# pingooio/pingoo

Hardware: AMD Instinct MI355X
Metric: requests/sec matched (whole node), 1k-rule WAF (higher is better)
Workload: dtype u8

## Files before the change

include/pwaf.h:

```cpp
#ifndef PWAF_H
#define PWAF_H

#include <stddef.h>
#include <stdint.h>

#ifdef __cplusplus
extern "C" {
#endif

#define PWAF_ABI_VERSION 4u

#define PWAF_OK 0
#define PWAF_E_INVALID_ARG (-1)
#define PWAF_E_SYNTAX (-2)
#define PWAF_E_UNSUPPORTED (-3)
#define PWAF_E_LIST (-4)
#define PWAF_E_DEVICE (-5)
#define PWAF_E_BATCH (-6)
#define PWAF_E_NOMEM (-7)
#define PWAF_E_BUSY (-8)
#define PWAF_W_PARTIAL 1

#define PWAF_ACTION_ALLOW 0u
#define PWAF_ACTION_BLOCK 1u
// ... 49 lines not shown
void pwaf_list_free(char **items, size_t n);

#define PWAF_OPT_NO_UA_GATE 1u
#define PWAF_OPT_NO_CAPTCHA_BYPASS 2u
#define PWAF_OPT_STRICT 8u
#define PWAF_OPT_LENIENT 32u
#define PWAF_OPT_GLOBAL_VERDICT_TABLES 128u
#define PWAF_OPT_SPARSE_VERDICT 16384u
#define PWAF_OPT_DENSE_VERDICT 2048u
#define PWAF_OPT_TINY_VERDICT_SLOTS 4096u
#define PWAF_OPT_NO_DENSE_SWITCH 65536u
#define PWAF_OPT_EAGER_CMP 32768u
#define PWAF_OPT_NO_DIR_SUMMARY 8192u
#define PWAF_OPT_GEO_ANSWERS 256u
#define PWAF_OPT_RULE_HITS 131072u
#define PWAF_OPT_NO_RESIDUAL 64u
#define PWAF_OPT_NO_RESIDUAL_JIT 1024u
#define PWAF_OPT_NO_PREFILTER 4u
#define PWAF_OPT_FILTER_STRIDE2 16u
#define PWAF_OPT_NO_CONFIRM 512u
typedef struct pwaf_options {
    uint32_t struct_size;
    uint32_t flags;
    int32_t device;
    uint32_t lds_table_budget;
    uint32_t max_dfa_states;
    uint32_t max_table_bytes;
    uint32_t reserved[2];
} pwaf_options;

// ... 238 lines not shown
int pwaf_engine_stats(const pwaf_engine *, pwaf_stats *out);
int pwaf_engine_rule_errors(pwaf_engine *, uint64_t *counts, size_t n_rules);
int pwaf_engine_residual_mode(const pwaf_engine *);
const char *pwaf_engine_residual_fallback(const pwaf_engine *);
size_t pwaf_program_residual_source(const pwaf_program *, int kind, char *buf, size_t cap);
long pwaf_program_residual_compile(const pwaf_program *, const char *arch, char *err, size_t err_len);
int pwaf_program_confirm_field(const pwaf_program *, uint32_t group, const uint8_t *bytes, size_t len, uint32_t arena_offset,
                               uint16_t *atoms, size_t cap, size_t *n_atoms, int *flagged, int *walk);
int pwaf_program_confirm_shape(const pwaf_program *, uint32_t group, uint32_t out[8]);
size_t pwaf_program_flat_image(const pwaf_program *, uint32_t group, uint32_t tier, uint8_t *buf, size_t cap);
#define PWAF_LIST_SCAN_WORDS 16
int pwaf_program_list_scans(const pwaf_program *, uint32_t *out, size_t cap, size_t *n_descs);
uint32_t pwaf_engine_compute_units(const pwaf_engine *);
int pwaf_engine_address_tables(const pwaf_engine *, uint32_t out[8]);
int pwaf_engine_coarse_tables(const pwaf_engine *, uint32_t out[16]);
int pwaf_program_stats(const pwaf_program *, pwaf_stats *out);

size_t pwaf_derive_path(const uint8_t *uri_path, size_t len);
void pwaf_derive_user_agent(const uint8_t *hdr, size_t len, int present, size_t *out_start, size_t *out_len);
void pwaf_derive_host(const uint8_t *uri_host, size_t uri_host_len, int uri_host_present,
                      const uint8_t *host_hdr, size_t host_hdr_len, int host_hdr_present,
                      int *out_from_header, size_t *out_start, size_t *out_len);

const char *pwaf_last_error(void);
uint32_t pwaf_abi_version(void);

#ifdef __cplusplus
}
#endif
#endif
// ... 1 lines not shown
```

pingoo_amd/_abi.py:

```python
import ctypes as C

ABI_VERSION = 4

OK = 0
E_INVALID_ARG = -1
E_SYNTAX = -2
E_UNSUPPORTED = -3
E_LIST = -4
E_DEVICE = -5
E_BATCH = -6
E_NOMEM = -7
E_BUSY = -8

ACTION_ALLOW, ACTION_BLOCK, ACTION_CAPTCHA, ACTION_BYPASS = 0, 1, 2, 3
RULE_NONE = 0xFFFFFFFF
RULE_UA_GATE = 0xFFFFFFFE
RULE_CAPTCHA_ENDPOINT = 0xFFFFFFFD
RULE_ACTION_BLOCK, RULE_ACTION_CAPTCHA = 1, 2

LIST_STRING, LIST_INT, LIST_IP = 0, 1, 2
OPT_NO_UA_GATE, OPT_NO_CAPTCHA_BYPASS, OPT_NO_PREFILTER, OPT_STRICT, OPT_FILTER_STRIDE2, OPT_LENIENT, OPT_NO_RESIDUAL, OPT_GLOBAL_VERDICT_TABLES, OPT_NO_CONFIRM, OPT_NO_RESIDUAL_JIT = 1, 2, 4, 8, 16, 32, 64, 128, 512, 1024
OPT_DENSE_VERDICT, OPT_TINY_VERDICT_SLOTS, OPT_NO_DIR_SUMMARY, OPT_SPARSE_VERDICT, OPT_EAGER_CMP, OPT_NO_DENSE_SWITCH = 2048, 4096, 8192, 16384, 32768, 65536
OPT_GEO_ANSWERS = 256
OPT_RULE_HITS = 131072
W_PARTIAL = 1
MEM_HOST, MEM_DEVICE = 0, 1
FLAG_CAPTCHA_VERIFIED = 1
ROUTE_NONE = 0xFFFFFFFF
RECORD_NONE = 0xFFFFFFFF
N_FIELDS = 5
FIELD_NAMES = ("host", "url", "path", "method", "user_agent")
ARENA_PAD = 16
ADDRESS_TABLE_FIELDS = ("escapes", "n_vals", "has_summary", "shift", "common", "packed", "classes", "sets")
CONFIRM_SHAPE_FIELDS = ("entries", "bytes", "class_words", "in_lds", "longest", "top_class_pos", "widest_bin", "has_walk")
LIST_SCAN_FIELDS = ("phase", "pass", "tier", "threads", "hot_bytes", "n_hot", "n_delta", "behind_filter", "merge_rec", "dense_mode", "share_owner", "need_bit",
                    "launch", "launch_count", "wg_per_cu", "zero15")
FLAT_SHAPE_FIELDS = ("n_states", "n_classes", "scalar_mode", "ill_class", "n_full", "n_delta", "lds_bytes")
COARSE_TABLE_FIELDS = ("present", "shift", "bytes", "blocks_set", "summary_blocks_set", "threads", "wg_per_cu", "zero7",
                       "rec_present", "rec_shift", "rec_bytes", "rec_blocks_set", "zero12", "zero13", "zero14", "zero15")
GEO_ANSWER_TABLE_FIELDS = ("has_table", "escapes", "n_vals", "has_summary", "shift", "common", "records", "zero")


class RuleDesc(C.Structure):
    _fields_ = [
        ("name", C.c_char_p),
        ("expression", C.c_char_p),
        ("actions", C.POINTER(C.c_uint8)),
        ("n_actions", C.c_uint32),
        ("reserved", C.c_uint32),
    ]


class RouteDesc(C.Structure):

# ... 201 lines not shown
```

pingoo_amd/csrc/engine.cpp:

```cpp
#include <hip/hip_runtime_api.h>

#include <cstdio>
#include <algorithm>
#include <cstring>
#include <map>
#include <memory>
#include <mutex>
#include <string>
#include <type_traits>
#include <unordered_map>
#include <vector>

#include "dirtable.h"
#include "georec.h"
#include "frontend.h"
#include "kernels.h"
#include "lscan_split.h"
#include "program.h"
#include "records.h"
#include "scanplan.h"
#include "tableplan.h"

using namespace pwaf;

// ... 157 lines not shown

struct Scratch {
    std::mutex mu;
    hipStream_t stream = nullptr, side = nullptr;
    hipEvent_t ev_fork = nullptr, ev_join = nullptr, done = nullptr;
    bool used = false;
    hipStream_t last = nullptr;
    bool last_own = false;
    DevBuf status;
    uint64_t pool_entries = 0;
    struct View { void *p = nullptr; };
    View res_cols;
    bool retry = false;
    DevBuf err_sink;
    DevBuf ipres;
    DevBuf rec, pool, gate_lists, attr;
    DevBuf verdict_spill;
    DevBuf res_words;
    DevBuf zero_block;
    View ctrl, cand_bits, visit_bits, walk_bits;
    DevBuf chunk_bits, cand_cnt;
    DevBuf need;
    DevBuf pairs;
    DevBuf zero_off;
    static constexpr uint32_t kArgSlots = 8;
    DevBuf args;
    PinBuf arg_slot[kArgSlots];
    hipEvent_t arg_ev[kArgSlots] = {};
    bool arg_pending[kArgSlots] = {};
    uint32_t arg_next = 0;
// ... 29 lines not shown
            if (ev) (void)hipEventDestroy(ev);
    }
};
static constexpr size_t kContexts = 3;

struct pwaf_engine : PlanShape, PassShape {
    pwaf_program prog;
    int device = 0;
    std::vector<std::unique_ptr<Scratch>> ctx;
    size_t next_ctx = 0;
    std::vector<DevGroup> groups;
    DevBuf num_atoms, bit_atoms , trig_off, trig_rules, always_rules, country_luts , rules, lits, set_masks;
    DevBuf lazy_atoms;
    DevBuf short_atoms;
    DevBuf class_rows, dir_esc, leaf_root, geo_leaf_root;
    DevBuf iu_vals[2], iu_masks[2];
    DevBuf ip_root4, ip_root6, ip_nodes, geo_root4, geo_root6, geo_nodes, geo_recs;
    std::mutex mu;
    std::mutex prof_mu;
    DevBuf residual_errors;
    std::string residual_note;
    JitKernel residual_jit;
    DevBuf rules_unrouted;
    DevBuf residual_blob, geo_rec_root4, geo_rec_root6, geo_rec_nodes;
    DevBuf pass_base, colmask, dir24 , dir_chunks, dir_vals, dir_summary;
    uint32_t dir_sum_shift = 0, dir_common = 0;
    DevBuf dir_coarse;
    uint32_t dir_coarse_shift = 0, dir_coarse_bytes = 0, dir_coarse_set = 0, dir_summary_set = 0;
    uint32_t dir_n_esc = 0, dir_n_vals = 0;
    bool geo_answers = false;
// ... 392 lines not shown
        v.always_rules = (const uint32_t *)e->always_rules.p;
        for (int var = 0; var < 2; var++) {
            v.iu_vals[var] = (const int64_t *)e->iu_vals[var].p;
            v.iu_masks[var] = (const uint32_t *)e->iu_masks[var].p;
            v.iu_n[var] = e->iu_n[var];
            v.iu_words[var] = e->iu_words[var];
        }
        v.country_masks = (const uint32_t *)e->country_luts.p;
        v.cc_words = e->cc_words;
        v.rules = (const DevRule *)e->rules.p;
        v.n_rules = (uint32_t)P.rules.size();
        v.lits = (const uint32_t *)e->lits.p;
        set_trie_args(e, v);
        if ((rc = S.ipres.reserve((size_t)n * (v.ipres_packed ? 4 : 8) + 64))) return rc;
        v.ipres = (uint32_t *)S.ipres.p;
        v.out = d_out;
        v.counts = (unsigned long long *)d_counts;
        v.match_idx = d_match_idx;
        v.n_matches = d_n_matches;
        return PWAF_OK;
    }

    int zero_head_records() {
        for (size_t k = 0; k < e->groups.size(); k++) {
            const DevGroup &d = e->groups[k];
            if (!d.filtered || d.filter.heads.empty()) continue;
            if (slab_count(col_bytes[d.field], slab0_of(d.field)) != 0 && !(sw.filter_debug_skip & 4u)) continue;
            HIP_TRY(hipMemsetAsync((uint32_t *)S.rec.p + k * (size_t)n, 0, (size_t)n * 4, stream));
        }
        return PWAF_OK;
// ... 28 lines not shown
        if (rc || !d_geo) return rc;
        GeoRecArgs ga{};
        set_georec_args(e, ga);
        ga.ip = db.ip;
        ga.ip_is_v6 = db.ip_is_v6;
        ga.asn = db.asn;
        ga.country = db.country;
        ga.n = n;
        ga.out = (uint2 *)d_geo;
        return side_stage(q, "georec", 25ull * n, "georec kernel", [&] { return launch_georec(ga, q); });
    }
    int attr_stage(hipStream_t q) {
        if (attr_launched) return PWAF_OK;
        attr_launched = true;
        if (q == stream && sw.placement == 0) HIP_TRY(hipStreamWaitEvent(stream, S.ev_join, 0));
        return side_stage(q, "attr", 0xFEu, "attribute kernel", [&] { return sw.skip_attr ? (int)hipMemsetAsync(v.ghdr, 0, (size_t)n_groups * 4, q) : launch_attr(v, q); });
    }
    int attr_at_start() {
        int rc;
        if (sw.placement == 0) return ipres_stage(S.side);
        if (sw.placement == 3) return (rc = ipres_stage(S.side)) ? rc : attr_stage(S.side);
        return PWAF_OK;
    }
    int attr_after_filter() {
        int rc;
        switch (sw.placement) {
        case 0: return attr_stage(stream);
        case 1: return (rc = ipres_stage(stream)) ? rc : attr_stage(stream);
        case 2: return (rc = ipres_stage(S.side)) ? rc : attr_stage(S.side);
        default: return PWAF_OK;
        }
// ... 662 lines not shown
    up(e->bit_atoms, t.bit_col);
    up(e->num_atoms, t.cmp_atoms);
    up(e->lazy_atoms, t.lazy_atoms);
    up(e->lits, t.lits);
    up(e->trig_off, t.trig_off);
    up(e->trig_rules, t.trig_rules);
    up(e->always_rules, t.always);
    up(e->country_luts, t.cc_masks);
    up(e->rules, P.rules);
    if (!t.rules_unrouted.empty()) up(e->rules_unrouted, t.rules_unrouted);
    up(e->set_masks, P.set_masks);
    up(e->ip_root4, P.ipset_trie.root4);
    up(e->ip_root6, P.ipset_trie.root6);
    up(e->ip_nodes, P.ipset_trie.nodes);
    up(e->class_rows, t.class_rows);
    up(e->geo_root4, t.geo_root4);
    up(e->geo_root6, t.geo_root6);
    up(e->geo_nodes, t.geo_nodes);
    up(e->leaf_root, std::vector<uint32_t>(65536, TRIE_LEAF));
    up(e->geo_leaf_root, std::vector<uint32_t>(65536, TRIE_LEAF | t.geo_default));
    if (P.n_residual) {
        up(e->residual_blob, P.residual_blob);
        up(e->residual_errors, std::vector<unsigned long long>(P.n_residual, 0ull));
        if (P.has_geo && P.residual_needs_geo) {
            const std::vector<uint32_t> leaf0(65536, TRIE_LEAF);
            up(e->geo_rec_root4, P.geo_trie.root4.empty() ? leaf0 : P.geo_trie.root4);
            up(e->geo_rec_root6, P.geo_trie.root6.empty() ? leaf0 : P.geo_trie.root6);
            up(e->geo_rec_nodes, P.geo_trie.nodes);
            up(e->geo_recs, P.geo_recs);
        }
// ... 241 lines not shown
    out[6] = e->n_classes;
    out[7] = P.set_words ? (uint32_t)(P.set_masks.size() / P.set_words) : 1u;
    return PWAF_OK;
}
int pwaf_engine_coarse_tables(const pwaf_engine *e, uint32_t out[16]) {
    if (!e || !out) return fail(PWAF_E_INVALID_ARG, "pwaf_engine_coarse_tables: NULL argument");
    const IpresShape sh = ipres_shape();
    for (int i = 0; i < 16; i++) out[i] = 0;
    out[0] = e->dir_coarse.p ? 1u : 0u;
    out[1] = e->dir_coarse_shift;
    out[2] = e->dir_coarse_bytes;
    out[3] = e->dir_coarse_set;
    out[4] = e->dir_summary_set;
    out[5] = e->dir_coarse.p ? sh.threads : 256u;
    out[6] = e->dir_coarse.p ? sh.wg_per_cu : 8u;
    return PWAF_OK;
}
int pwaf_engine_geo_answer_tables(const pwaf_engine *e, uint32_t out[8]) {
    if (!e || !out) return fail(PWAF_E_INVALID_ARG, "pwaf_engine_geo_answer_tables: NULL argument");
    if (int rc = need_geo_answers(e, "pwaf_engine_geo_answer_tables")) return rc;
    out[0] = e->georec_chunks.p ? 1u : 0u;
    out[1] = e->georec_n_esc;
    out[2] = e->georec_chunks.p ? e->georec_n_vals : 0u;
    out[3] = e->georec_summary.p ? 1u : 0u;
    out[4] = e->georec_shift;
    out[5] = e->georec_common;
    out[6] = (uint32_t)std::max<size_t>(1, e->prog.p->geo_recs.size());
    out[7] = 0;
    return PWAF_OK;
}
// ... 864 lines not shown
```

pingoo_amd/csrc/kernels.h:

```cpp
#pragma once
#include <cstdint>
#include <string>
#include <vector>

#include "program.h"
#include "scanplan.h"

namespace pwaf {

static constexpr int kMaxPasses = 250;
static constexpr int kVerdictPre = 12;
static constexpr uint32_t kDirChunkWords = 32;

static constexpr uint32_t REC_OVERFLOW = 0x80000000u;
struct PoolEntry {
    uint32_t atom;
    uint32_t next;
};

struct ScanArgs {
    const uint8_t *data;
    const uint32_t *off;
    uint32_t n;
    const uint16_t *tab;
// ... 282 lines not shown
    const uint32_t *dir_summary;
    uint32_t dir_sum_shift, dir_common;
    const uint32_t *dir_coarse;
    uint32_t dir_coarse_shift, dir_coarse_bytes;
    const uint2 *dir_esc;
    const uint32_t *class_rows;
    uint32_t class_words;
    uint32_t acmp_words;
    uint32_t geo_default;
    uint32_t *ipres;
    uint32_t ipres_packed;
    uint32_t has_geo;
    uint4 *gpairs;
    uint32_t *ghdr;
    uint32_t pair_stride;
    uint32_t attr_blocks;
    pwaf_verdict *out;
    unsigned long long *counts;
    uint32_t *match_idx;
    uint32_t *n_matches;
    pwaf_rule_hit *hits;
    uint32_t hits_cap;
    uint32_t *n_hits;
    unsigned long long *rule_hits;
    uint32_t *route;
    uint32_t route_base;
};

int launch_scan(const ScanArgs &a, void *stream);
struct GatedTable {
// ... 36 lines not shown
```

pingoo_amd/csrc/kernels.hip:

```cpp
#include <hip/hip_runtime.h>

#include <cstdlib>
#include <mutex>
#include <set>

#include "confirm.h"
#include "utf8.h"
#include "kernels.h"
#include "residual.h"

namespace pwaf {

static constexpr int kScanThreads = 1024;
static constexpr int kScanWaves = kScanThreads / 64;
static constexpr uint32_t kNone = 0xFFFFFFFFu;

#define PWAF_LDS __attribute__((address_space(3)))
#define PWAF_GLOBAL __attribute__((address_space(1)))
typedef const PWAF_LDS uint16_t *lds_u16_ptr;
typedef const PWAF_GLOBAL uint16_t *glb_u16_ptr;
typedef const PWAF_LDS uint32_t *lds_u32_ptr;
typedef const PWAF_LDS uint8_t *lds_u8_ptr;
typedef unsigned int u32x4 __attribute__((ext_vector_type(4)));
typedef u32x4 u32x4_u __attribute__((aligned(1)));
// ... 2271 lines not shown

    constexpr int kPre = BR == 1 ? 4 : kVerdictPre;
    constexpr int kBitRegs = BR;
    struct Bits {
        unsigned long long w[kBitRegs];
    };
    struct Inputs {
        uint32_t rv[kPre];
        uint32_t base[kPre];
        Bits bits;
        unsigned long long rest[kBitRegs];
        uint32_t flags, n_pairs;
        uint4 pair0;
        uint32_t res0;
        uint32_t lraw[2];
    };
    const uint32_t *my_bits[kBitRegs];
    uint32_t my_base[kBitRegs];
    bool my_live[kBitRegs];
#pragma unroll
    for (int r = 0; r < kBitRegs; r++) {
        const uint32_t ps = (uint32_t)r * 64 + lane;
        my_live[r] = ps < a.n_passes;
        my_bits[r] = nullptr;
        my_base[r] = 0;
        if (my_live[r]) {
            const PassInfo pi = a.passes[ps];
            const uint32_t kind = pi.kind_slot >> 24, sl = pi.kind_slot & 0xFFFFFFu;
            if (kind == 3) my_live[r] = false;
            my_bits[r] = kind == 1 ? a.cand_bits + (size_t)sl * a.bit_words : kind == 2 ? a.visit_bits + (size_t)sl * a.bit_words : nullptr;
// ... 23 lines not shown
                if (ps == kNone && nzp[r] != 0) {
                    const int l = __builtin_ctzll(nzp[r]);
                    nzp[r] &= nzp[r] - 1;
                    ps = (uint32_t)r * 64 + (uint32_t)l;
                    word = ((unsigned long long)(uint32_t)__builtin_amdgcn_readlane((int)(bt.w[r] >> 32), l) << 32) | (uint32_t)__builtin_amdgcn_readlane((int)(uint32_t)bt.w[r], l);
                    base = (uint32_t)__builtin_amdgcn_readlane((int)my_base[r], l);
                }
            }
            in.base[q] = base;
            in.rv[q] = (ps != kNone && valid && ((word >> lane) & 1ull)) ? a.rec[(size_t)ps * a.n + i] : 0u;
        }
#pragma unroll
        for (int r = 0; r < kBitRegs; r++) in.rest[r] = nzp[r];
        in.bits = bt;
        in.flags = valid ? (uint32_t)a.flags[i] : 0u;
        const uint32_t gg = min(g, a.n_groups - 1);
        {
            const uint32_t *src = a.ghdr + gg;
#pragma unroll
            for (uint32_t sl = 0; sl < 2; sl++) {
                if (sl >= a.n_lazy_var) break;
                const uint32_t vi = a.lazy_var[sl];
                if (vi != 5u && lane == 1u + sl) src = (vi < 5u ? a.off[vi] : a.hoff[vi - 7u]) + gg * 64u;
            }
            in.n_pairs = *src;
        }
        in.pair0 = a.gpairs[(size_t)gg * a.pair_stride + lane];
        in.res0 = (a.res_words && valid) ? a.res_match[i] : 0u;
        in.lraw[0] = in.lraw[1] = 0u;
        const uint32_t ii = valid ? i : 0u;
// ... 22 lines not shown
    for (uint32_t g = blockIdx.x * n_waves + wave; g < a.n_groups; g += g_stride) {
        const uint32_t i = g * 64 + lane;
        const bool valid = i < a.n;
        const unsigned long long valid_mask = __ballot(valid);
        Inputs nxt;
        request_inputs(g + g_stride, b_nxt, nxt);
        request_bits(g + 2 * g_stride, b_nxt);

        for (uint32_t k = lane; k < rulew; k += 64) rulebm[k] = k < 64 ? h_always : a.always_rules[k];
        __builtin_amdgcn_fence(__ATOMIC_ACQ_REL, "wavefront");

        const uint32_t flags = cur.flags;
        const uint4 *pairs = a.gpairs + (size_t)g * a.pair_stride;
        const uint32_t n_pairs = (uint32_t)__builtin_amdgcn_readlane((int)cur.n_pairs, 0);
        const unsigned long long verified_mask = __ballot(valid && (flags & PWAF_FLAG_CAPTCHA_VERIFIED));

        uint32_t n_entries = 1;
        auto triggers = [&](const uint32_t c) {
            if (dbg_skip & 8u) return;
            const uint32_t kb = LT ? (uint32_t)l_trig_off[c] : a.trig_off[c], ke = LT ? (uint32_t)l_trig_off[c + 1] : a.trig_off[c + 1];
            for (uint32_t k = kb; k < ke; k++) {
                const uint32_t r = LT ? (uint32_t)l_trig_rules[k] : (uint32_t)a.trig_rules[k];
                atomicOr(&rulebm[r >> 5], 1u << (r & 31));
            }
        };
        if (true_triggers && lane == 0) triggers(0);
        auto append_batch = [&](const uint32_t c, const uint32_t lo, const uint32_t hi, const uint32_t cnt) {
            if (lane < cnt) {
                const uint32_t e = n_entries + lane;
                const unsigned long long m = ((unsigned long long)hi << 32) | lo;
// ... 138 lines not shown
            const uint32_t word = wb + lane < rulew ? rulebm[wb + lane] : 0u;
            const uint32_t pc = (uint32_t)__builtin_popcount(word), incl = wave_scan_add(pc);
            uint32_t pos = n_cand + incl - pc, wrd = word;
            while (wrd) {
                cand[pos++] = (uint16_t)((wb + lane) * 32 + (uint32_t)__builtin_ctz(wrd));
                wrd &= wrd - 1;
            }
            n_cand += (uint32_t)__builtin_amdgcn_readlane((int)incl, 63);
        }
        __builtin_amdgcn_fence(__ATOMIC_ACQ_REL, "wavefront");

        unsigned long long pending = valid_mask;
        uint32_t n_exact = 0;
        bool undecided = valid;
        uint32_t my_action = PWAF_ACTION_ALLOW, my_rule = PWAF_RULE_NONE;
        unsigned long long gated = 0;
        unsigned long long rpending = ROUTES ? valid_mask : 0ull;
        uint32_t my_route = PWAF_ROUTE_NONE;
        for (uint32_t base = 0; base < n_cand && (HITS || pending != 0 || (ROUTES && rpending != 0)) && !(dbg_skip & 32u); base += 64) {
            unsigned long long fire = 0, eff_mask = 0;
            unsigned long long match = 0;
            uint32_t lit_off = 0, lit_cnt = 0;
            bool lazy_seen = false;
            bool is_route = false;
            if (base + lane < n_cand) {
                const uint32_t my_cand = cand[base + lane];
                if (ROUTES) is_route = my_cand >= a.route_base;
                uint32_t eff_u, eff_v;
                if (LT) {
                    const uint2 hdr = l_rules[my_cand];
// ... 78 lines not shown
            unsigned long long rfiring = 0;
            if (ROUTES) {
                const unsigned long long rlanes = __ballot(is_route);
                rfiring = firing & rlanes;
                firing &= ~rlanes;
            }
            uint32_t first = kNone;
            while (firing != 0 && pending != 0) {
                const int j = __builtin_ctzll(firing);
                firing &= firing - 1;
                const unsigned long long fj = (((unsigned long long)(uint32_t)__builtin_amdgcn_readlane((int)(uint32_t)(fire >> 32), j) << 32) |
                                               (uint32_t)__builtin_amdgcn_readlane((int)(uint32_t)fire, j)) & pending;
                if (fj & mybit) first = (uint32_t)j;
                pending &= ~fj;
            }
            if (undecided && first != kNone) {
                undecided = false;
                const uint32_t jc = cand[base + first];
                uint32_t eff_u, eff_v;
                if (LT) {
                    const uint32_t y = l_rules[jc].y;
                    eff_u = (y >> 16) & 0xFFu;
                    eff_v = y >> 24;
                    const uint32_t pi = l_pub[jc];
                    my_rule = pi >= 0xFFF0u ? 0xFFFF0000u | pi : pi;
                } else {
                    const DevRule dr = a.rules[jc];
                    eff_u = dr.eff_unverified;
                    eff_v = dr.eff_verified;
                    my_rule = dr.public_idx;
                }
// ... 30 lines not shown
                        if (q_n == 0) {
                            q_g0 = g;
                            q_k = 0;
                        }
                        for (; has != 0; has &= has - 1) {
                            const int j = __builtin_ctzll(has);
                            const unsigned long long wj = ((unsigned long long)(uint32_t)__builtin_amdgcn_readlane((int)(uint32_t)(word >> 32), j) << 32) |
                                                          (uint32_t)__builtin_amdgcn_readlane((int)(uint32_t)word, j);
                            park96(q_rk, q_lo, q_hi, (uint32_t)__builtin_amdgcn_readlane((int)pub, j) | (q_k << 16), wj, q_n);
                            q_n++;
                        }
                    }
                }
            }
        }
        if (dbg_skip & 512u) my_rule = n_exact;
        if (dbg_skip & 64u) my_rule = n_cand | (n_entries << 16);

        if (valid) {
            uint2 v;
            v.x = my_action;
            v.y = my_rule;
            *reinterpret_cast<uint2 *>(&a.out[i]) = v;
            if (ROUTES) a.route[i] = my_route;
        }
        const unsigned long long m_block = __ballot(valid && my_action == PWAF_ACTION_BLOCK);
        const unsigned long long m_captcha = __ballot(valid && my_action == PWAF_ACTION_CAPTCHA);
        const unsigned long long m_bypass = __ballot(valid && my_action == PWAF_ACTION_BYPASS);
        cnt_block += (unsigned)__builtin_popcountll(m_block);
        cnt_captcha += (unsigned)__builtin_popcountll(m_captcha);
// ... 301 lines not shown
    const bool from_row = a.asn == nullptr;
#ifdef PWAF_PROFILING
    const bool skip_rows = (a.debug_skip >> 18) & 1u, skip_transpose = (a.debug_skip >> 19) & 1u, skip_cmp = (a.debug_skip >> 20) & 1u;
#else
    constexpr bool skip_rows = false, skip_transpose = false, skip_cmp = false;
#endif
    uint32_t h_col = 0, h_c = 0;
    if (lane < a.n_cmp) {
        h_col = a.cmp[lane].col;
        h_c = a.cmp[lane].c;
    }
    const uint32_t g_stride = gridDim.x * 4;
    const uint32_t *const asn_col = from_row ? a.off[0] : a.asn;
    const uint16_t *const country_col = from_row ? a.port : a.country;
    const uint32_t *const short_col = a.n_short ? a.short_off : a.off[0];
    const uint8_t *const short_bytes = a.n_short ? a.short_data : reinterpret_cast<const uint8_t *>(a.off[0]);
    auto load_in = [&](const uint32_t g, AttrIn &in) {
        const uint32_t i0 = g * 64 + lane;
        const uint32_t i = (g < a.n_groups && i0 < a.n) ? i0 : 0u;
        if (PACKED) {
            const uint32_t w = a.ipres[i];
            in.cls = w & 0xFFFFu;
            in.set_id = w >> 16;
        } else {
            const uint2 w = reinterpret_cast<const uint2 *>(a.ipres)[i];
            in.cls = w.x;
            in.set_id = w.y;
        }
        in.port = a.port[i];
#pragma unroll
// ... 72 lines not shown
                if (a.iu_vals[var][mid] < v) lo = mid + 1;
                else hi = mid;
            }
            if (lo < a.iu_n[var] && a.iu_vals[var][lo] == v) r_int[var] = lo + 1;
        }
        const uint32_t *srow = a.set_masks + (size_t)set_id * a.set_words;
        const uint32_t *crow = from_row ? a.class_rows + (size_t)cls * a.class_words : a.country_masks + (size_t)r_geo * a.cc_words;
        const uint32_t *prow = a.iu_masks[0] + (size_t)r_int[0] * a.iu_words[0];
        const uint32_t *arow = from_row ? crow + a.cc_words : a.iu_masks[1] + (size_t)r_int[1] * a.iu_words[1];
        const uint32_t *qrow = crow + a.cc_words + a.iu_words[1];
        const bool rows_on = valid && !skip_rows;
        const bool have_s = rows_on && a.n_ip_lists && set_id, have_c = rows_on && (from_row ? cls != 0 : true), have_p = rows_on && r_int[0],
                   have_a = rows_on && (from_row ? cls != 0 : r_int[1] != 0), have_q = rows_on && from_row && cls != 0;
        uint32_t rs[SW], rc[CW], rp[IW], ra[IW], rq[QW];
#pragma unroll
        for (uint32_t q = 0; q < SW; q++) rs[q] = (q < a.set_words && have_s) ? srow[q] : 0u;
#pragma unroll
        for (uint32_t q = 0; q < CW; q++) rc[q] = (q < a.cc_words && have_c) ? crow[q] : 0u;
#pragma unroll
        for (uint32_t q = 0; q < IW; q++) rp[q] = (q < a.iu_words[0] && have_p) ? prow[q] : 0u;
#pragma unroll
        for (uint32_t q = 0; q < IW; q++) ra[q] = (q < a.iu_words[1] && have_a) ? arow[q] : 0u;
#pragma unroll
        for (uint32_t q = 0; q < QW; q++) rq[q] = (q < a.acmp_words && have_q) ? qrow[q] : 0u;

        AttrIn nn;
        load_in(g + 2 * g_stride, nn);
        uint32_t n_slo, n_shi;
        load_short(nxt, n_slo, n_shi);
#pragma unroll
        for (uint32_t q = 0; q < SW; q++) asm volatile("" : "+v"(rs[q]));
#pragma unroll
        for (uint32_t q = 0; q < CW; q++) asm volatile("" : "+v"(rc[q]));
#pragma unroll
        for (uint32_t q = 0; q < IW; q++) asm volatile("" : "+v"(rp[q]), "+v"(ra[q]));
#pragma unroll
        for (uint32_t q = 0; q < QW; q++) asm volatile("" : "+v"(rq[q]));

        auto transpose = [&](const uint32_t w, const uint32_t slot) {
            const uint32_t orw0 = wave_or(w);
            if (orw0 == 0) return;
            uint32_t mine_lo = 0, mine_hi = 0;
            for (uint32_t orw = orw0; orw; orw &= orw - 1) {
                const uint32_t b = (uint32_t)__builtin_ctz(orw);
                const unsigned long long m = __ballot((w & (1u << b)) != 0u);
                park64(mine_lo, mine_hi, m, b);
            }
            const bool owner = lane < 32 && ((orw0 >> lane) & 1u);
            const uint32_t c = owner ? tab[slot * 32 + (lane & 31u)] : 0u;
            emit_pairs(c != 0, c, mine_lo, mine_hi);
        };
        if (!skip_transpose) {
#pragma unroll
            for (uint32_t q = 0; q < SW; q++) if (q < a.set_words) transpose(rs[q], q);
#pragma unroll
            for (uint32_t q = 0; q < CW; q++) if (q < a.cc_words) transpose(rc[q], kSlotCc + q);
#pragma unroll
            for (uint32_t q = 0; q < IW; q++) if (q < a.iu_words[0]) transpose(rp[q], kSlotPort + q);
#pragma unroll
            for (uint32_t q = 0; q < IW; q++) if (q < a.iu_words[1]) transpose(ra[q], kSlotAsn + q);
#pragma unroll
            for (uint32_t q = 0; q < QW; q++) if (q < a.acmp_words) transpose(rq[q], kSlotAcmp + q);
        }

        for (uint32_t base = 0; base < a.n_cmp && !skip_cmp; base += 64) {
            uint32_t m_col = h_col, m_c = h_c;
            if (base != 0) {
                m_col = m_c = 0;
                if (base + lane < a.n_cmp) {
                    if (base < 64 + kAttrCmpStaged) {
                        m_col = tab[kLdsCmp + 2 * (base - 64 + lane)];
                        m_c = tab[kLdsCmp + 2 * (base - 64 + lane) + 1];
                    } else {
                        m_col = a.cmp[base + lane].col;
                        m_c = a.cmp[base + lane].c;
                        asm volatile("" : "+v"(m_col), "+v"(m_c));
                    }
// ... 290 lines not shown
```

pingoo_amd/csrc/tableplan.cpp:

```cpp
#include "tableplan.h"

#include <algorithm>
#include <map>
#include <string>

namespace pwaf {

int fail(int code, const std::string &msg);

namespace {

struct Canon { uint32_t vi, op, col, c; };

int merge_int_sets(const Program &P, std::vector<NumAtomDev> &atoms, TablePlan &out) {
    for (int var = 0; var < 2; var++) {
        std::map<int64_t, std::vector<uint32_t>> member;
        uint32_t n_sets = 0;
        for (auto &d : atoms) {
            if (d.kind != ATOM_INTSET || d.var != var) continue;
            for (uint32_t k = d.ref; k < d.ref2; k++) member[P.int_pool[k]].push_back(n_sets);
            d.ref = n_sets++;
        }
        if (n_sets > 32 * kIntWordsMax) return fail(PWAF_E_UNSUPPORTED, "more than 128 integer-set predicates on one client variable");
        const uint32_t words = out.iu_words[var] = std::max(1u, (n_sets + 31) / 32);
// ... 216 lines not shown
        auto ins = class_of.emplace(row, (uint32_t)class_of.size());
        if (ins.second) out.class_rows.insert(out.class_rows.end(), row.begin(), row.end());
        rec_class[r] = ins.first->second;
    }
    out.n_classes = (uint32_t)class_of.size();
    out.geo_default = rec_class[0];
    auto remap = [&](const std::vector<uint32_t> &src) {
        std::vector<uint32_t> leaves(src);
        for (auto &x : leaves)
            if (x & TRIE_LEAF) x = TRIE_LEAF | rec_class[x & ~TRIE_LEAF];
        return leaves;
    };
    out.geo_root4 = remap(P.geo_trie.root4);
    out.geo_root6 = remap(P.geo_trie.root6);
    out.geo_nodes = remap(P.geo_trie.nodes);
}

}

int plan_tables(const Program &P, size_t n_rules, size_t n_routes, TablePlan &out) {
    out = TablePlan();
    std::vector<NumAtomDev> atoms = P.num_atoms;
    if (int rc = merge_int_sets(P, atoms, out)) return rc;
    if (P.n_cols >= (1u << 20)) return fail(PWAF_E_UNSUPPORTED, "more than 2^20 predicate columns");
    if (P.set_words > kSetWordsMax) return fail(PWAF_E_UNSUPPORTED, "more than 512 ip lists");
    if (P.country_luts.size() > 32 * kCcWordsMax) return fail(PWAF_E_UNSUPPORTED, "more than 256 distinct client.country predicates");
    std::vector<uint32_t> bit_atoms;
    std::vector<NumAtomDev> cmp_src;
    split_atoms(atoms, bit_atoms, cmp_src);
    out.n_bit_atoms = (uint32_t)bit_atoms.size();
// ... 3 lines not shown
    if (int rc = canonical_comparisons(cmp_src, out.hlen_fields, canon)) return rc;
    const std::vector<uint8_t> flipped = choose_polarity(P, canon);
    const std::vector<uint32_t> L = flip_literals(P.lits, flipped);
    if (int rc = encode_comparisons(canon, flipped, out)) return rc;
    if (P.rules.size() > 65519 || n_rules + n_routes > 65519) return fail(PWAF_E_UNSUPPORTED, n_routes ? "more than 65519 rules and routes" : "more than 65519 rules");
    const TriggerUse use = trigger_lists(P, L, rarity_ranks(P, cmp_src, bit_atoms), out);
    const std::vector<uint32_t> lazy_of = select_lazy(P, use, out);
    out.n_cmp_atoms = (uint32_t)out.cmp_atoms.size();
    for (const CmpAtomDev &ca : out.cmp_atoms) out.cmp_vars |= 1u << std::min(31u, cmp_code_var(ca.col >> 24));
    out.n_lazy = (uint32_t)out.lazy_atoms.size();
    if (out.lazy_atoms.empty()) out.lazy_atoms.push_back({0, 0});
    out.lits = device_literals(L, lazy_of);
    transpose_countries(P, out);
    out.rules_unrouted = unrouted_rules(P);
    record_classes(P, out);
    return PWAF_OK;
}

}
```

pingoo_amd/csrc/tableplan.h:

```cpp
#pragma once
#include <cstdint>
#include <utility>
#include <vector>

#include "program.h"

namespace pwaf {

inline uint32_t verdict_mode(uint32_t flags) {
    const bool tiny = (flags & PWAF_OPT_TINY_VERDICT_SLOTS) != 0;
    if (flags & PWAF_OPT_DENSE_VERDICT) return 0u;
    if (flags & PWAF_OPT_SPARSE_VERDICT) return tiny ? 2u : 1u;
    return tiny ? 4u : 3u;
}

static constexpr uint32_t kCmpComplement = 0x80u, kCmpVarAsn = 6u, kCmpVarHeader = 7u;
inline uint32_t cmp_code(uint32_t var, uint32_t op, bool complement) { return (2u * var + op) | (complement ? kCmpComplement : 0u); }
inline uint32_t cmp_code_var(uint32_t code) { return (code & 0x7Fu) / 2u; }

struct PlanShape {
    uint32_t iu_n[2] = {0, 0}, iu_words[2] = {1, 1};
    uint32_t n_bit_atoms = 0;
    uint32_t n_cmp_atoms = 0, cmp_vars = 0;
    uint32_t n_lazy = 0;
    std::vector<uint32_t> lazy_vars;
    std::vector<uint32_t> hlen_fields;
    uint32_t n_trig = 0;
    uint32_t cc_words = 1, acmp_words = 0;
    uint32_t class_words = 1, n_classes = 1, geo_default = 0;
};

struct TablePlan : PlanShape {
    std::vector<int64_t> iu_vals[2];
    std::vector<uint32_t> iu_masks[2];
    std::vector<uint32_t> bit_col;
    std::vector<CmpAtomDev> cmp_atoms;
    std::vector<CmpAtomDev> lazy_atoms;
    std::vector<uint32_t> lits;
    std::vector<uint32_t> trig_off;
    std::vector<uint16_t> trig_rules;
    std::vector<uint32_t> always;
    std::vector<uint32_t> cc_masks;
    std::vector<std::pair<uint32_t, uint32_t>> acmp;
    std::vector<uint32_t> class_rows;
    std::vector<uint32_t> geo_root4, geo_root6, geo_nodes;
    std::vector<DevRule> rules_unrouted;
};

int plan_tables(const Program &P, size_t n_rules, size_t n_routes, TablePlan &out);

}
```

pingoo_amd/engine.py:

```python
from __future__ import annotations

import ctypes as C
import enum
import ipaddress
import os
from dataclasses import dataclass, field
from typing import Dict, Iterable, List, Optional, Sequence, Tuple

import numpy as np

from . import _abi
from .batch import GEO_DTYPE, RULE_HIT_DTYPE, VERDICT_DTYPE, Request, RequestBatch

_LIB = None
_LIB_PATH = os.path.join(os.path.dirname(os.path.abspath(__file__)), f"libpwaf_{os.environ['PWAF_LIB_VARIANT']}.so" if os.environ.get("PWAF_LIB_VARIANT") else "libpwaf.so")


class PwafError(RuntimeError):
    def __init__(self, code: int, message: str, rule_index: Optional[int] = None):
        super().__init__(f"[{code}] {message}")
        self.code = code
        self.message = message
        self.rule_index = rule_index

# ... 120 lines not shown
    L.pwaf_program_compile_routed.argtypes = routed_args + [C.POINTER(vp), C.POINTER(_abi.CompileError)]
    L.pwaf_engine_create_routed.argtypes = routed_args + [C.POINTER(vp), C.POINTER(_abi.CompileError)]
    for fn_name in ("pwaf_engine_route_count", "pwaf_program_route_count"):
        getattr(L, fn_name).argtypes = [vp]
        getattr(L, fn_name).restype = C.c_uint32
    L.pwaf_evaluate_batch_routes.argtypes = [vp, C.POINTER(_abi.Batch), vp, vp, vp]
    L.pwaf_evaluate_device_routes.argtypes = [vp, C.POINTER(_abi.Batch), vp, vp, vp, vp, vp, vp]
    L.pwaf_evaluate_one_route.argtypes = [vp, C.POINTER(_abi.Request), C.POINTER(_abi.Verdict), C.POINTER(C.c_uint32)]
    L.pwaf_evaluate_records_geo.argtypes = [vp, vp, C.c_size_t, vp, C.c_uint32, vp, vp, vp]
    L.pwaf_evaluate_one_geo.argtypes = [vp, C.POINTER(_abi.Request), C.POINTER(_abi.Verdict), C.POINTER(_abi.Geo)]
    L.pwaf_async_create_geo.argtypes = [vp, C.c_uint32, C.c_uint32, C.c_uint32, C.POINTER(vp)]
    L.pwaf_async_poll_geo.argtypes = [vp, C.POINTER(_abi.Completion), C.POINTER(_abi.Geo), C.c_size_t]
    L.pwaf_async_poll_geo.restype = C.c_size_t
    L.pwaf_engine_geo_answer_tables.argtypes = [vp, C.POINTER(C.c_uint32)]
    L.pwaf_engine_coarse_tables.argtypes = [vp, C.POINTER(C.c_uint32)]
    L.pwaf_geoip_from_mmdb.argtypes = [C.c_char_p, C.c_size_t, C.POINTER(C.POINTER(_abi.GeoipEntry)), C.POINTER(C.c_size_t)]
    L.pwaf_geoip_from_file_image.argtypes = [C.c_char_p, C.c_char_p, C.c_size_t, C.POINTER(C.POINTER(_abi.GeoipEntry)), C.POINTER(C.c_size_t)]
    L.pwaf_zstd_decompress.argtypes = [C.c_char_p, C.c_size_t, C.POINTER(C.c_void_p), C.POINTER(C.c_size_t)]
    L.pwaf_buffer_free.argtypes = [C.c_void_p]
    L.pwaf_buffer_free.restype = None
    L.pwaf_geoip_free.argtypes = [C.POINTER(_abi.GeoipEntry)]
    L.pwaf_geoip_free.restype = None
    L.pwaf_list_parse_csv.argtypes = [C.c_char_p, C.c_size_t, C.POINTER(C.POINTER(C.c_char_p)), C.POINTER(C.c_size_t)]
    L.pwaf_list_free.argtypes = [C.POINTER(C.c_char_p), C.c_size_t]
    L.pwaf_list_free.restype = None
    L.pwaf_engine_kernel_times.argtypes = [vp, C.POINTER(_abi.KernelTime), C.c_int]
    L.pwaf_derive_path.argtypes = [C.c_char_p, C.c_size_t]
    L.pwaf_derive_path.restype = C.c_size_t
    L.pwaf_derive_user_agent.argtypes = [C.c_char_p, C.c_size_t, C.c_int, C.POINTER(C.c_size_t), C.POINTER(C.c_size_t)]
    L.pwaf_derive_user_agent.restype = None
# ... 259 lines not shown
        return int(lib().pwaf_engine_compute_units(self._h))

    def address_tables(self) -> dict:
        out = (C.c_uint32 * len(_abi.ADDRESS_TABLE_FIELDS))()
        rc = lib().pwaf_engine_address_tables(self._h, out)
        if rc != 0:
            _raise(rc, lib().pwaf_last_error().decode(errors="replace"))
        return dict(zip(_abi.ADDRESS_TABLE_FIELDS, (int(x) for x in out)))

    def coarse_tables(self) -> dict:
        out = (C.c_uint32 * len(_abi.COARSE_TABLE_FIELDS))()
        rc = lib().pwaf_engine_coarse_tables(self._h, out)
        if rc != 0:
            _raise(rc, lib().pwaf_last_error().decode(errors="replace"))
        return dict(zip(_abi.COARSE_TABLE_FIELDS, (int(x) for x in out)))

    def geo_answer_tables(self) -> dict:
        out = (C.c_uint32 * len(_abi.GEO_ANSWER_TABLE_FIELDS))()
        rc = lib().pwaf_engine_geo_answer_tables(self._h, out)
        if rc != 0:
            _raise(rc, lib().pwaf_last_error().decode(errors="replace"))
        return dict(zip(_abi.GEO_ANSWER_TABLE_FIELDS, (int(x) for x in out)))

    def lookup_geoip(self, ip16, v6) -> np.ndarray:
        ip16 = np.ascontiguousarray(ip16, dtype=np.uint8).reshape(-1, 16)
        v6 = np.ascontiguousarray(v6, dtype=np.uint8).reshape(-1)
        assert len(ip16) == len(v6)
        out = np.zeros(len(v6), dtype=GEO_DTYPE)
        rc = lib().pwaf_geoip_lookup(self._h, ip16.ctypes.data, v6.ctypes.data, len(v6), _abi.MEM_HOST, out.ctypes.data, None)
        if rc != 0:
# ... 636 lines not shown
```

Measured before the change: 7.862 billion.

## Precompute per-set and per-class rule floors to skip attribute-only columns

At compile time, attribute columns that only appear as the lone positive first literal of a rule term are found. For each IP set and geo class, the lowest-index rule they trigger is folded into a floor table, split into verified and unverified halves. The attribute kernel writes a per-request floor instead of transposing those bitmask words, dropping or skipping those words. The verdict kernel takes the minimum of the first matched rule and the floor, then resolves the action once after the loop. This removes transpose and compare work for such columns and defers rule lookup, at the cost of an extra per-request buffer, extra loads, and a more complex verdict path limited to the non-hits, non-routes case.

```diff
diff --git a/include/pwaf.h b/include/pwaf.h
--- a/include/pwaf.h
+++ b/include/pwaf.h
@@ -87,6 +87,7 @@
 #define PWAF_OPT_NO_DIR_SUMMARY 8192u
 #define PWAF_OPT_GEO_ANSWERS 256u
 #define PWAF_OPT_RULE_HITS 131072u
+#define PWAF_OPT_NO_ATTR_FLOOR 262144u
 #define PWAF_OPT_NO_RESIDUAL 64u
 #define PWAF_OPT_NO_RESIDUAL_JIT 1024u
 #define PWAF_OPT_NO_PREFILTER 4u
@@ -355,6 +356,7 @@
 uint32_t pwaf_engine_compute_units(const pwaf_engine *);
 int pwaf_engine_address_tables(const pwaf_engine *, uint32_t out[8]);
 int pwaf_engine_coarse_tables(const pwaf_engine *, uint32_t out[16]);
+int pwaf_engine_floor_tables(const pwaf_engine *, uint32_t out[8]);
 int pwaf_program_stats(const pwaf_program *, pwaf_stats *out);
 
 size_t pwaf_derive_path(const uint8_t *uri_path, size_t len);
diff --git a/pingoo_amd/_abi.py b/pingoo_amd/_abi.py
--- a/pingoo_amd/_abi.py
+++ b/pingoo_amd/_abi.py
@@ -23,6 +23,7 @@
 OPT_DENSE_VERDICT, OPT_TINY_VERDICT_SLOTS, OPT_NO_DIR_SUMMARY, OPT_SPARSE_VERDICT, OPT_EAGER_CMP, OPT_NO_DENSE_SWITCH = 2048, 4096, 8192, 16384, 32768, 65536
 OPT_GEO_ANSWERS = 256
 OPT_RULE_HITS = 131072
+OPT_NO_ATTR_FLOOR = 262144
 W_PARTIAL = 1
 MEM_HOST, MEM_DEVICE = 0, 1
 FLAG_CAPTCHA_VERIFIED = 1
@@ -38,6 +39,7 @@
 FLAT_SHAPE_FIELDS = ("n_states", "n_classes", "scalar_mode", "ill_class", "n_full", "n_delta", "lds_bytes")
 COARSE_TABLE_FIELDS = ("present", "shift", "bytes", "blocks_set", "summary_blocks_set", "threads", "wg_per_cu", "zero7",
                        "rec_present", "rec_shift", "rec_bytes", "rec_blocks_set", "zero12", "zero13", "zero14", "zero15")
+FLOOR_TABLE_FIELDS = ("floor_cols", "floor_words", "skipped_words", "skipped_words_own_geo", "set_entries", "class_entries", "zero6", "zero7")
 GEO_ANSWER_TABLE_FIELDS = ("has_table", "escapes", "n_vals", "has_summary", "shift", "common", "records", "zero")
 
 
diff --git a/pingoo_amd/csrc/engine.cpp b/pingoo_amd/csrc/engine.cpp
--- a/pingoo_amd/csrc/engine.cpp
+++ b/pingoo_amd/csrc/engine.cpp
@@ -195,6 +195,7 @@
     bool retry = false;
     DevBuf err_sink;
     DevBuf ipres;
+    DevBuf afloor;
     DevBuf rec, pool, gate_lists, attr;
     DevBuf verdict_spill;
     DevBuf res_words;
@@ -254,6 +255,7 @@
     DevBuf lazy_atoms;
     DevBuf short_atoms;
     DevBuf class_rows, dir_esc, leaf_root, geo_leaf_root;
+    DevBuf set_floor, class_floor;
     DevBuf iu_vals[2], iu_masks[2];
     DevBuf ip_root4, ip_root6, ip_nodes, geo_root4, geo_root6, geo_nodes, geo_recs;
     std::mutex mu;
@@ -676,6 +678,17 @@
         set_trie_args(e, v);
         if ((rc = S.ipres.reserve((size_t)n * (v.ipres_packed ? 4 : 8) + 64))) return rc;
         v.ipres = (uint32_t *)S.ipres.p;
+        v.set_floor = (const uint32_t *)e->set_floor.p;
+        v.class_floor = db.asn == nullptr ? (const uint32_t *)e->class_floor.p : nullptr;
+        if (v.set_floor || v.class_floor) {
+            if ((rc = S.afloor.reserve((size_t)n * 4))) return rc;
+            v.afloor = (uint32_t *)S.afloor.p;
+            for (uint32_t s = 0; s < kSrcWords; s++) {
+                if (!(s < kSrcCc ? v.set_floor != nullptr : v.class_floor != nullptr)) continue;
+                v.floor_drop[s] = e->floor_mask[s];
+                if (e->floor_mask[s] && !(e->floor_used[s] & ~e->floor_mask[s])) v.floor_skip |= 1ull << s;
+            }
+        }
         v.out = d_out;
         v.counts = (unsigned long long *)d_counts;
         v.match_idx = d_match_idx;
@@ -734,7 +747,11 @@
         if (attr_launched) return PWAF_OK;
         attr_launched = true;
         if (q == stream && sw.placement == 0) HIP_TRY(hipStreamWaitEvent(stream, S.ev_join, 0));
-        return side_stage(q, "attr", 0xFEu, "attribute kernel", [&] { return sw.skip_attr ? (int)hipMemsetAsync(v.ghdr, 0, (size_t)n_groups * 4, q) : launch_attr(v, q); });
+        return side_stage(q, "attr", 0xFEu, "attribute kernel", [&] {
+            if (!sw.skip_attr) return launch_attr(v, q);
+            if (v.afloor) (void)hipMemsetAsync(v.afloor, 0xFF, (size_t)n * 4, q);
+            return (int)hipMemsetAsync(v.ghdr, 0, (size_t)n_groups * 4, q);
+        });
     }
     int attr_at_start() {
         int rc;
@@ -1427,6 +1444,8 @@
     up(e->ip_root6, P.ipset_trie.root6);
     up(e->ip_nodes, P.ipset_trie.nodes);
     up(e->class_rows, t.class_rows);
+    if (!t.set_floor.empty()) up(e->set_floor, t.set_floor);
+    if (!t.class_floor.empty()) up(e->class_floor, t.class_floor);
     up(e->geo_root4, t.geo_root4);
     up(e->geo_root6, t.geo_root6);
     up(e->geo_nodes, t.geo_nodes);
@@ -1698,6 +1717,21 @@
     out[4] = e->dir_summary_set;
     out[5] = e->dir_coarse.p ? sh.threads : 256u;
     out[6] = e->dir_coarse.p ? sh.wg_per_cu : 8u;
+    return PWAF_OK;
+}
+int pwaf_engine_floor_tables(const pwaf_engine *e, uint32_t out[8]) {
+    if (!e || !out) return fail(PWAF_E_INVALID_ARG, "pwaf_engine_floor_tables: NULL argument");
+    for (int i = 0; i < 8; i++) out[i] = 0;
+    out[0] = e->n_floor_cols;
+    for (uint32_t s = 0; s < kSrcWords && s < e->floor_mask.size(); s++) {
+        if (!e->floor_mask[s]) continue;
+        const bool all = !(e->floor_used[s] & ~e->floor_mask[s]);
+        out[1]++;
+        out[2] += all ? 1u : 0u;
+        out[3] += (all && s < kSrcCc) ? 1u : 0u;
+    }
+    out[4] = (uint32_t)(e->set_floor.p ? (e->prog.p->set_words ? std::max<size_t>(1, e->prog.p->set_masks.size() / e->prog.p->set_words) : 1) : 0);
+    out[5] = e->class_floor.p ? e->n_classes : 0u;
     return PWAF_OK;
 }
 int pwaf_engine_geo_answer_tables(const pwaf_engine *e, uint32_t out[8]) {
diff --git a/pingoo_amd/csrc/kernels.h b/pingoo_amd/csrc/kernels.h
--- a/pingoo_amd/csrc/kernels.h
+++ b/pingoo_amd/csrc/kernels.h
@@ -320,6 +320,10 @@
     uint4 *gpairs;
     uint32_t *ghdr;
     uint32_t pair_stride;
+    const uint32_t *set_floor, *class_floor;
+    uint32_t *afloor;
+    uint32_t floor_drop[kSrcWords];
+    unsigned long long floor_skip;
     uint32_t attr_blocks;
     pwaf_verdict *out;
     unsigned long long *counts;
diff --git a/pingoo_amd/csrc/kernels.hip b/pingoo_amd/csrc/kernels.hip
--- a/pingoo_amd/csrc/kernels.hip
+++ b/pingoo_amd/csrc/kernels.hip
@@ -2309,6 +2309,7 @@
         uint4 pair0;
         uint32_t res0;
         uint32_t lraw[2];
+        uint32_t afloor;
     };
     const uint32_t *my_bits[kBitRegs];
     uint32_t my_base[kBitRegs];
@@ -2362,6 +2363,12 @@
         for (int r = 0; r < kBitRegs; r++) in.rest[r] = nzp[r];
         in.bits = bt;
         in.flags = valid ? (uint32_t)a.flags[i] : 0u;
+        in.afloor = 0xFFFFFFFFu;
+        if (!HITS && !ROUTES) {
+            const bool fl = a.afloor != nullptr;
+            const uint32_t w = (fl ? a.afloor : a.ghdr)[(fl && valid) ? i : 0u];
+            in.afloor = (fl && valid) ? w : 0xFFFFFFFFu;
+        }
         const uint32_t gg = min(g, a.n_groups - 1);
         {
             const uint32_t *src = a.ghdr + gg;
@@ -2414,6 +2421,7 @@
         const uint4 *pairs = a.gpairs + (size_t)g * a.pair_stride;
         const uint32_t n_pairs = (uint32_t)__builtin_amdgcn_readlane((int)cur.n_pairs, 0);
         const unsigned long long verified_mask = __ballot(valid && (flags & PWAF_FLAG_CAPTCHA_VERIFIED));
+        const uint32_t my_floor = (flags & PWAF_FLAG_CAPTCHA_VERIFIED) ? cur.afloor >> 16 : cur.afloor & 0xFFFFu;
 
         uint32_t n_entries = 1;
         auto triggers = [&](const uint32_t c) {
@@ -2582,6 +2590,7 @@
         uint32_t n_exact = 0;
         bool undecided = valid;
         uint32_t my_action = PWAF_ACTION_ALLOW, my_rule = PWAF_RULE_NONE;
+        uint32_t my_dev = 0xFFFFu;
         unsigned long long gated = 0;
         unsigned long long rpending = ROUTES ? valid_mask : 0ull;
         uint32_t my_route = PWAF_ROUTE_NONE;
@@ -2690,7 +2699,12 @@
                 if (fj & mybit) first = (uint32_t)j;
                 pending &= ~fj;
             }
-            if (undecided && first != kNone) {
+            if (!HITS && !ROUTES) {
+                if (undecided && first != kNone) {
+                    undecided = false;
+                    my_dev = cand[base + first];
+                }
+            } else if (undecided && first != kNone) {
                 undecided = false;
                 const uint32_t jc = cand[base + first];
                 uint32_t eff_u, eff_v;
@@ -2751,6 +2765,25 @@
                 }
             }
         }
+        if (!HITS && !ROUTES) {
+            my_dev = min(my_dev, my_floor);
+            if (valid && my_dev != 0xFFFFu) {
+                uint32_t eff_u, eff_v;
+                if (LT) {
+                    const uint32_t y = l_rules[my_dev].y;
+                    eff_u = (y >> 16) & 0xFFu;
+                    eff_v = y >> 24;
+                    const uint32_t pi = l_pub[my_dev];
+                    my_rule = pi >= 0xFFF0u ? 0xFFFF0000u | pi : pi;
+                } else {
+                    const DevRule dr = a.rules[my_dev];
+                    eff_u = dr.eff_unverified;
+                    eff_v = dr.eff_verified;
+                    my_rule = dr.public_idx;
+                }
+                my_action = (verified_mask & mybit) ? eff_v : eff_u;
+            }
+        }
         if (dbg_skip & 512u) my_rule = n_exact;
         if (dbg_skip & 64u) my_rule = n_cand | (n_entries << 16);
 
@@ -3082,6 +3115,9 @@
     const uint32_t *const asn_col = from_row ? a.off[0] : a.asn;
     const uint16_t *const country_col = from_row ? a.port : a.country;
     const uint32_t *const short_col = a.n_short ? a.short_off : a.off[0];
+    const bool fl_set = a.set_floor != nullptr, fl_cls = a.class_floor != nullptr;
+    const uint32_t *const sfl_tab = fl_set ? a.set_floor : a.bit_col, *const cfl_tab = fl_cls ? a.class_floor : a.bit_col;
+    auto skipped = [&](const uint32_t src) { return ((a.floor_skip >> src) & 1ull) != 0ull; };
     const uint8_t *const short_bytes = a.n_short ? a.short_data : reinterpret_cast<const uint8_t *>(a.off[0]);
     auto load_in = [&](const uint32_t g, AttrIn &in) {
         const uint32_t i0 = g * 64 + lane;
@@ -3184,15 +3220,16 @@
                    have_a = rows_on && (from_row ? cls != 0 : r_int[1] != 0), have_q = rows_on && from_row && cls != 0;
         uint32_t rs[SW], rc[CW], rp[IW], ra[IW], rq[QW];
 #pragma unroll
-        for (uint32_t q = 0; q < SW; q++) rs[q] = (q < a.set_words && have_s) ? srow[q] : 0u;
-#pragma unroll
-        for (uint32_t q = 0; q < CW; q++) rc[q] = (q < a.cc_words && have_c) ? crow[q] : 0u;
+        for (uint32_t q = 0; q < SW; q++) rs[q] = (q < a.set_words && !skipped(kSrcSet + q) && have_s) ? srow[q] : 0u;
+#pragma unroll
+        for (uint32_t q = 0; q < CW; q++) rc[q] = (q < a.cc_words && !skipped(kSrcCc + q) && have_c) ? crow[q] : 0u;
 #pragma unroll
         for (uint32_t q = 0; q < IW; q++) rp[q] = (q < a.iu_words[0] && have_p) ? prow[q] : 0u;
 #pragma unroll
-        for (uint32_t q = 0; q < IW; q++) ra[q] = (q < a.iu_words[1] && have_a) ? arow[q] : 0u;
-#pragma unroll
-        for (uint32_t q = 0; q < QW; q++) rq[q] = (q < a.acmp_words && have_q) ? qrow[q] : 0u;
+        for (uint32_t q = 0; q < IW; q++) ra[q] = (q < a.iu_words[1] && !skipped(kSrcAsn + q) && have_a) ? arow[q] : 0u;
+#pragma unroll
+        for (uint32_t q = 0; q < QW; q++) rq[q] = (q < a.acmp_words && !skipped(kSrcAcmp + q) && have_q) ? qrow[q] : 0u;
+        uint32_t f_set = sfl_tab[(fl_set && valid) ? set_id : 0u], f_cls = cfl_tab[(fl_cls && valid) ? cls : 0u];
 
         AttrIn nn;
         load_in(g + 2 * g_stride, nn);
@@ -3206,6 +3243,20 @@
         for (uint32_t q = 0; q < IW; q++) asm volatile("" : "+v"(rp[q]), "+v"(ra[q]));
 #pragma unroll
         for (uint32_t q = 0; q < QW; q++) asm volatile("" : "+v"(rq[q]));
+        asm volatile("" : "+v"(f_set), "+v"(f_cls));
+        if (fl_set || fl_cls) {
+            if (!(fl_set && valid)) f_set = 0xFFFFFFFFu;
+            if (!(fl_cls && valid)) f_cls = 0xFFFFFFFFu;
+            if (valid) a.afloor[i] = min(f_set & 0xFFFFu, f_cls & 0xFFFFu) | (min(f_set >> 16, f_cls >> 16) << 16);
+        }
+#pragma unroll
+        for (uint32_t q = 0; q < SW; q++) rs[q] &= ~a.floor_drop[kSrcSet + q];
+#pragma unroll
+        for (uint32_t q = 0; q < CW; q++) rc[q] &= ~a.floor_drop[kSrcCc + q];
+#pragma unroll
+        for (uint32_t q = 0; q < IW; q++) ra[q] &= ~a.floor_drop[kSrcAsn + q];
+#pragma unroll
+        for (uint32_t q = 0; q < QW; q++) rq[q] &= ~a.floor_drop[kSrcAcmp + q];
 
         auto transpose = [&](const uint32_t w, const uint32_t slot) {
             const uint32_t orw0 = wave_or(w);
@@ -3222,15 +3273,15 @@
         };
         if (!skip_transpose) {
 #pragma unroll
-            for (uint32_t q = 0; q < SW; q++) if (q < a.set_words) transpose(rs[q], q);
-#pragma unroll
-            for (uint32_t q = 0; q < CW; q++) if (q < a.cc_words) transpose(rc[q], kSlotCc + q);
+            for (uint32_t q = 0; q < SW; q++) if (q < a.set_words && !skipped(kSrcSet + q)) transpose(rs[q], q);
+#pragma unroll
+            for (uint32_t q = 0; q < CW; q++) if (q < a.cc_words && !skipped(kSrcCc + q)) transpose(rc[q], kSlotCc + q);
 #pragma unroll
             for (uint32_t q = 0; q < IW; q++) if (q < a.iu_words[0]) transpose(rp[q], kSlotPort + q);
 #pragma unroll
-            for (uint32_t q = 0; q < IW; q++) if (q < a.iu_words[1]) transpose(ra[q], kSlotAsn + q);
-#pragma unroll
-            for (uint32_t q = 0; q < QW; q++) if (q < a.acmp_words) transpose(rq[q], kSlotAcmp + q);
+            for (uint32_t q = 0; q < IW; q++) if (q < a.iu_words[1] && !skipped(kSrcAsn + q)) transpose(ra[q], kSlotAsn + q);
+#pragma unroll
+            for (uint32_t q = 0; q < QW; q++) if (q < a.acmp_words && !skipped(kSrcAcmp + q)) transpose(rq[q], kSlotAcmp + q);
         }
 
         for (uint32_t base = 0; base < a.n_cmp && !skip_cmp; base += 64) {
diff --git a/pingoo_amd/csrc/tableplan.cpp b/pingoo_amd/csrc/tableplan.cpp
--- a/pingoo_amd/csrc/tableplan.cpp
+++ b/pingoo_amd/csrc/tableplan.cpp
@@ -254,6 +254,70 @@
     out.geo_root4 = remap(P.geo_trie.root4);
     out.geo_root6 = remap(P.geo_trie.root6);
     out.geo_nodes = remap(P.geo_trie.nodes);
+}
+
+void floor_tables(const Program &P, const std::vector<uint32_t> &L, TablePlan &out) {
+    out.floor_mask.assign(kSrcWords, 0);
+    out.floor_used.assign(kSrcWords, 0);
+    for (uint32_t k = 0; k < kSrcWords * 32; k++)
+        if (out.bit_col[k]) out.floor_used[k >> 5] |= 1u << (k & 31);
+    if ((P.flags & (PWAF_OPT_RULE_HITS | PWAF_OPT_NO_ATTR_FLOOR)) || P.n_routes || P.n_dev_routes || verdict_mode(P.flags) < 3u) return;
+    std::vector<uint32_t> n_occ(P.n_cols, 0), n_pure(P.n_cols, 0);
+    auto each_pure = [&](auto &&fn) {
+        for (size_t r = 0; r < P.rules.size(); r++) {
+            const DevRule &dr = P.rules[r];
+            uint32_t first = dr.lit_off;
+            for (uint32_t k = dr.lit_off; k < dr.lit_off + dr.lit_cnt; k++) {
+                if (!(L[k] & LIT_TERM_END)) continue;
+                if (k == first && !(L[k] & LIT_NEG)) fn((uint32_t)r, L[k] & LIT_ATOM_MASK);
+                first = k + 1;
+            }
+        }
+    };
+    for (const DevRule &dr : P.rules)
+        for (uint32_t k = dr.lit_off; k < dr.lit_off + dr.lit_cnt; k++) n_occ[L[k] & LIT_ATOM_MASK]++;
+    each_pure([&](uint32_t, uint32_t c) { n_pure[c]++; });
+    std::vector<uint8_t> floor_only(P.n_cols, 0);
+    for (uint32_t k = 0; k < kSrcWords * 32; k++) {
+        const uint32_t c = out.bit_col[k], src = k >> 5;
+        if (c == 0 || (src >= kSrcPort && src < kSrcAsn) || n_occ[c] == 0 || n_occ[c] != n_pure[c]) continue;
+        out.floor_mask[src] |= 1u << (k & 31);
+        if (!floor_only[c]) out.n_floor_cols++;
+        floor_only[c] = 1;
+    }
+    if (out.n_floor_cols == 0) return;
+    std::vector<uint32_t> col_floor(P.n_cols, 0xFFFFFFFFu);
+    each_pure([&](uint32_t r, uint32_t c) {
+        if (!floor_only[c]) return;
+        uint32_t lo = col_floor[c] & 0xFFFFu, hi = col_floor[c] >> 16;
+        if (P.rules[r].eff_unverified) lo = std::min(lo, r);
+        if (P.rules[r].eff_verified) hi = std::min(hi, r);
+        col_floor[c] = lo | (hi << 16);
+    });
+    auto fold = [&](uint32_t &f, uint32_t word, uint32_t src) {
+        for (uint32_t w = word & out.floor_mask[src]; w; w &= w - 1) {
+            const uint32_t cf = col_floor[out.bit_col[src * 32 + (uint32_t)__builtin_ctz(w)]];
+            f = std::min(f & 0xFFFFu, cf & 0xFFFFu) | (std::min(f >> 16, cf >> 16) << 16);
+        }
+    };
+    bool any_set = false, any_class = false;
+    for (uint32_t s = 0; s < kSrcWords; s++) (s < kSrcCc ? any_set : any_class) |= out.floor_mask[s] != 0;
+    if (any_set) {
+        const size_t n_sets = P.set_words ? P.set_masks.size() / P.set_words : 0;
+        out.set_floor.assign(std::max<size_t>(1, n_sets), 0xFFFFFFFFu);
+        for (size_t s = 0; s < n_sets; s++)
+            for (uint32_t w = 0; w < P.set_words; w++) fold(out.set_floor[s], P.set_masks[s * P.set_words + w], kSrcSet + w);
+    }
+    if (any_class) {
+        out.class_floor.assign(out.n_classes, 0xFFFFFFFFu);
+        const uint32_t iw = out.iu_words[1];
+        for (uint32_t c = 0; c < out.n_classes; c++) {
+            const uint32_t *row = &out.class_rows[(size_t)c * out.class_words];
+            for (uint32_t w = 0; w < out.cc_words; w++) fold(out.class_floor[c], row[w], kSrcCc + w);
+            for (uint32_t w = 0; w < iw; w++) fold(out.class_floor[c], row[out.cc_words + w], kSrcAsn + w);
+            for (uint32_t w = 0; w < out.acmp_words; w++) fold(out.class_floor[c], row[out.cc_words + iw + w], kSrcAcmp + w);
+        }
+    }
 }
 
 }
@@ -287,6 +351,7 @@
     transpose_countries(P, out);
     out.rules_unrouted = unrouted_rules(P);
     record_classes(P, out);
+    floor_tables(P, L, out);
     return PWAF_OK;
 }
 
diff --git a/pingoo_amd/csrc/tableplan.h b/pingoo_amd/csrc/tableplan.h
--- a/pingoo_amd/csrc/tableplan.h
+++ b/pingoo_amd/csrc/tableplan.h
@@ -28,6 +28,8 @@
     uint32_t n_trig = 0;
     uint32_t cc_words = 1, acmp_words = 0;
     uint32_t class_words = 1, n_classes = 1, geo_default = 0;
+    std::vector<uint32_t> floor_mask, floor_used;
+    uint32_t n_floor_cols = 0;
 };
 
 struct TablePlan : PlanShape {
@@ -44,6 +46,7 @@
     std::vector<std::pair<uint32_t, uint32_t>> acmp;
     std::vector<uint32_t> class_rows;
     std::vector<uint32_t> geo_root4, geo_root6, geo_nodes;
+    std::vector<uint32_t> set_floor, class_floor;
     std::vector<DevRule> rules_unrouted;
 };
 
diff --git a/pingoo_amd/engine.py b/pingoo_amd/engine.py
--- a/pingoo_amd/engine.py
+++ b/pingoo_amd/engine.py
@@ -158,6 +158,7 @@
     L.pwaf_async_poll_geo.restype = C.c_size_t
     L.pwaf_engine_geo_answer_tables.argtypes = [vp, C.POINTER(C.c_uint32)]
     L.pwaf_engine_coarse_tables.argtypes = [vp, C.POINTER(C.c_uint32)]
+    L.pwaf_engine_floor_tables.argtypes = [vp, C.POINTER(C.c_uint32)]
     L.pwaf_geoip_from_mmdb.argtypes = [C.c_char_p, C.c_size_t, C.POINTER(C.POINTER(_abi.GeoipEntry)), C.POINTER(C.c_size_t)]
     L.pwaf_geoip_from_file_image.argtypes = [C.c_char_p, C.c_char_p, C.c_size_t, C.POINTER(C.POINTER(_abi.GeoipEntry)), C.POINTER(C.c_size_t)]
     L.pwaf_zstd_decompress.argtypes = [C.c_char_p, C.c_size_t, C.POINTER(C.c_void_p), C.POINTER(C.c_size_t)]
@@ -447,6 +448,13 @@
         if rc != 0:
             _raise(rc, lib().pwaf_last_error().decode(errors="replace"))
         return dict(zip(_abi.COARSE_TABLE_FIELDS, (int(x) for x in out)))
+
+    def floor_tables(self) -> dict:
+        out = (C.c_uint32 * len(_abi.FLOOR_TABLE_FIELDS))()
+        rc = lib().pwaf_engine_floor_tables(self._h, out)
+        if rc != 0:
+            _raise(rc, lib().pwaf_last_error().decode(errors="replace"))
+        return dict(zip(_abi.FLOOR_TABLE_FIELDS, (int(x) for x in out)))
 
     def geo_answer_tables(self) -> dict:
         out = (C.c_uint32 * len(_abi.GEO_ANSWER_TABLE_FIELDS))()
```

Measured after the change: 7.718 billion. 0.982x the previous value.
